# gabefreedman/fastfp

Hardware: NVIDIA H100
Metric: Fp evals/sec (freqs x pulsars x draws) (higher is better)
Workload: dtype f64

## Files before the change

fastfp_b200/csrc/ffp_internal.cuh:

```cuda
#pragma once
#include <cuda_runtime.h>
#include <stdint.h>

#include <atomic>
#include <map>
#include <memory>
#include <string>
#include <type_traits>
#include <vector>

#include "../../include/fastfp_b200.h"

namespace ffp {

constexpr int NWC = 8;
constexpr int NWP = 16;
constexpr int NTC = NWC * 32, NTP = NWP * 32;
constexpr int CTAS_PER_SM = 1;
constexpr int CONSUMER_REGS = 120, PRODUCER_REGS = 56;
constexpr int VST = 16;
constexpr int FLUSH_TOAS = 512;
constexpr int MAX_M = 640;
constexpr int RG_ROWS = 288;
constexpr int MAX_M_WIDE = 2688;
constexpr int MAX_RG = (MAX_M_WIDE + RG_ROWS - 1) / RG_ROWS;

__host__ __device__ inline int row_groups(int m) { return m <= MAX_M ? 1 : (m + RG_ROWS - 1) / RG_ROWS; }
__host__ __device__ inline int row_group_start(int m, int k) {
  const int nb = (m + 7) / 8, g = row_groups(m);
  const int r = 8 * (k * (nb / g) + (k < nb % g ? k : nb % g));
  return r < m ? r : m;
}

inline int sweep_rows(int m, int64_t R, bool blockn) {
  return (m + 7) / 8 * 8 + (int)((R + 7) / 8 * 8) + (blockn ? 8 : 0);
}

template <int NMBW_, int NNB_, int WMW_, int CI_, int NWC_ = ffp::NWC, int NWP_ = ffp::NWP,
          int CREGS_ = CONSUMER_REGS, int PREGS_ = PRODUCER_REGS>
struct SweepCfg {
  static constexpr int NMBW = NMBW_, NNB = NNB_, WMW = WMW_, CI = CI_;
  static constexpr int NWC = NWC_, NWP = NWP_, NTC = NWC_ * 32, NTP = NWP_ * 32, NTHREADS = NTC + NTP;
  static constexpr int CREGS = CREGS_, PREGS = PREGS_;
  static_assert(NTHREADS <= 1024 && NWC % WMW_ == 0, "warp layout");
  static_assert(NTC * CREGS + NTP * PREGS <= NTHREADS * ((65536 / NTHREADS) / 8 * 8), "register pool");
  static constexpr int WNW = NWC / WMW;
  static constexpr int KF = WNW * NNB * 4;
  static constexpr int NMB = NMBW * WMW;
  static constexpr int MP = 8 * NMB;
  static constexpr int KB = CI / 4;
  static constexpr int ST = CI * 2 * KF;
  static constexpr int VEC = 4 * CI;
  static constexpr int GT = CI * MP;
  static constexpr int PK = VEC + GT;
  static constexpr int NX = KF / 8;
  static constexpr int XW = NX >= NWP ? NX / NWP : 1;
  static constexpr int KSPLIT = NX >= ffp::NWP ? 1 : (ffp::NWP / NX < KB ? ffp::NWP / NX : KB);
  static constexpr int KBW = KB / KSPLIT;
  static constexpr int WPG = NX >= NWP ? 1 : (NWP / NX < KSPLIT ? NWP / NX : KSPLIT);
  static constexpr int SPW = KSPLIT / WPG;
  static constexpr int NACTIVE = NX >= NWP ? NWP : NX * WPG;
  static constexpr int NV = PREGS >= 72 ? KBW * XW : 1;
  static constexpr int NACC = 2 * NMBW * NNB;
  static constexpr int NACCX = NACC + 3 * NNB;
  static constexpr int SLAB = NACCX * NTC + 5 * SPW * XW * NTP;
  static constexpr int FLUSH = FLUSH_TOAS / CI;
  static constexpr int SST = ST * 8 * 8 <= 140 * 1024 ? 8 : 4;
  static constexpr int GBUDGET = 214 * 1024 - SST * ST * 8 - VST * VEC * 8;
  static constexpr int GST = GBUDGET / (GT * 8) >= 8 ? 8 : (GBUDGET / (GT * 8) >= 2 ? GBUDGET / (GT * 8) : 2);
  static constexpr int RED = KF * (3 * WMW + 5 * KSPLIT);
  static constexpr size_t SMEM =
      (size_t)(SST * ST + GST * GT + VST * VEC + KF + RED + 2 * (SST + GST + VST)) * 8 + 128;
  static_assert(KB % KSPLIT == 0 && KSPLIT % WPG == 0 && NACTIVE <= NWP && (KBW * XW) % NV == 0,
                "basis-phase mapping");
  static_assert(GST >= 3, "the consumers prefetch across chunk boundaries: three G stages at least");
};

__host__ __device__ inline int g_frag_index(int il, int j, int nmb) {
  return (((il >> 2) * nmb + (j >> 3)) << 5) + (((j & 7) << 2) | (il & 3));
}

struct PulsarMeta {
  int64_t pk_off;
  int64_t L_off;
  int64_t raw_off;
  int64_t T_off;
  int32_t n, m, nch, mpad;
  int32_t mfix, mvar;
  int32_t var_off;
  int32_t ci;
  double tabs_max;
  int64_t dm_off;
  int64_t i8_off;
  int32_t i8_rows;
  int32_t i8_nst;
  double ninv_sum;
};
constexpr int RG_WIDE = 4;

struct KernelCfg {
  int nmbw, nnb, wmw, ci;
  int nwc = NWC;
  int kf() const { return (nwc / wmw) * nnb * 4; }
  int mp() const { return 8 * nmbw * wmw; }
  bool operator<(const KernelCfg& o) const {
    if (nmbw != o.nmbw) return nmbw < o.nmbw;
// ... 260 lines not shown
               const double* dx, const double* dy, const double* dx0, double* d_work, double* d_out,
               cudaStream_t st);
int run_fp64_peak(int kind, int iters, double* tflops, double* ms);

__device__ __forceinline__ uint32_t smem_u32(const void* p) {
  return (uint32_t)__cvta_generic_to_shared(p);
}
__device__ __forceinline__ void mbar_init(uint64_t* bar, int count) {
  asm volatile("mbarrier.init.shared::cta.b64 [%0], %1;" ::"r"(smem_u32(bar)), "r"(count));
}
__device__ __forceinline__ void mbar_expect_tx(uint64_t* bar, uint32_t bytes) {
  asm volatile("mbarrier.arrive.expect_tx.shared::cta.b64 _, [%0], %1;" ::"r"(smem_u32(bar)),
               "r"(bytes)
               : "memory");
}
__device__ __forceinline__ void tma_load_1d(void* dst_smem, const void* src_gmem, uint32_t bytes,
                                            uint64_t* bar) {
  asm volatile(
      "cp.async.bulk.shared::cluster.global.mbarrier::complete_tx::bytes [%0], [%1], %2, [%3];" ::
          "r"(smem_u32(dst_smem)),
      "l"(src_gmem), "r"(bytes), "r"(smem_u32(bar))
      : "memory");
}
__device__ __forceinline__ bool mbar_try_wait(uint64_t* bar, uint32_t parity) {
  uint32_t ok;
  asm volatile(
      "{\n .reg .pred p;\n mbarrier.try_wait.parity.shared::cta.b64 p, [%1], %2;\n"
      " selp.b32 %0, 1, 0, p;\n}"
      : "=r"(ok)
      : "r"(smem_u32(bar)), "r"(parity)
      : "memory");
  return ok != 0;
}
__device__ __forceinline__ void mbar_wait(uint64_t* bar, uint32_t parity) {
  if (mbar_try_wait(bar, parity)) return;
  while (!mbar_try_wait(bar, parity)) __nanosleep(64);
}
__device__ __forceinline__ void mbar_wait_spin(uint64_t* bar, uint32_t parity) {
  while (!mbar_try_wait(bar, parity)) {}
}
__device__ __forceinline__ void mbar_arrive(uint64_t* bar) {
  asm volatile("mbarrier.arrive.shared::cta.b64 _, [%0];" ::"r"(smem_u32(bar)) : "memory");
}
__device__ __forceinline__ void fence_barrier_init() {
  asm volatile("fence.mbarrier_init.release.cluster;" ::: "memory");
}
__device__ __forceinline__ void fence_proxy_async() {
  asm volatile("fence.proxy.async.shared::cta;" ::: "memory");
}

template <int R>
__device__ __forceinline__ void reg_alloc() {
  asm volatile("setmaxnreg.inc.sync.aligned.u32 %0;" ::"n"(R));
}
template <int R>
__device__ __forceinline__ void reg_dealloc() {
  asm volatile("setmaxnreg.dec.sync.aligned.u32 %0;" ::"n"(R));
}

__device__ __forceinline__ void dmma_m8n8k4(double& d0, double& d1, double a, double b) {
  asm("mma.sync.aligned.m8n8k4.row.col.f64.f64.f64.f64 {%0,%1}, {%2}, {%3}, {%0,%1};"
      : "+d"(d0), "+d"(d1)
      : "d"(a), "d"(b));
}
__device__ __forceinline__ void dmma_m16n8k4(double (&d)[4], double a0, double a1, double b) {
  asm("mma.sync.aligned.m16n8k4.row.col.f64.f64.f64.f64 {%0,%1,%2,%3}, {%4,%5}, {%6}, {%0,%1,%2,%3};"
// ... 124 lines not shown
```

fastfp_b200/csrc/fp_sweep_kernel.cuh:

```cuda
#pragma once
#include "ffp_internal.cuh"
#include "ffp_sincos.cuh"

namespace ffp {

enum class SweepMode { Fp, Nmfp, Res };

struct SweepArgs {
  const double* packets;
  const PulsarMeta* meta;
  const int* pidx;
  int ntile_f;
  int nwork;
  const double* freqs;
  int64_t F;
  union {
    FpOut fp;
    NmfpTiles nm;
    ResOut res;
  };
  RowGroupOut rg;
  double* slab;
  unsigned int* counter;
  const unsigned char* done_mask;
// ... 6 lines not shown
#else
#define FFP_DBG(ar, bit) 0
#endif

template <class C>
struct SweepSmem {
  double* Sring;
  double* Gring;
  double* Vring;
  double* fq;
  double* red;
  uint64_t *s_full, *s_empty, *g_full, *g_empty, *v_full, *v_empty;
  __device__ explicit SweepSmem(unsigned char* raw) {
    Sring = reinterpret_cast<double*>(raw);
    Gring = Sring + C::SST * C::ST;
    Vring = Gring + C::GST * C::GT;
    fq = Vring + VST * C::VEC;
    red = fq + C::KF;
    s_full = reinterpret_cast<uint64_t*>(red + C::RED);
    s_empty = s_full + C::SST;
    g_full = s_empty + C::SST;
    g_empty = g_full + C::GST;
    v_full = g_empty + C::GST;
    v_empty = v_full + VST;
  }
};

struct WorkItem {
  int p, ft, nch;
  const double* gpk;
};

template <class C>
__device__ __forceinline__ void producer_loop(const SweepArgs& ar, SweepSmem<C>& sm, volatile int* s_work,
                                              const int pw, const int lane) {
  constexpr int XW = C::XW, SPW = C::SPW, KBW = C::KBW, NV = C::NV;
  const int tidp = pw * 32 + lane;
  const int bk = lane & 3, bf8 = lane >> 2;
  const int bx0 = C::NX >= C::NWP ? pw * XW : pw % C::NX;
  const int bsplit = C::NX >= C::NWP ? 0 : (pw / C::NX) * SPW;
  const int sofs = 2 * lane;
  double* const sl = ar.slab + (size_t)blockIdx.x * C::SLAB + (size_t)C::NACCX * C::NTC + tidp;
  uint32_t g = 0;
  for (;;) {
    __syncthreads();
    const int w = *s_work;
    if (w >= ar.nwork) break;
    const int gp = w / ar.ntile_f;
    const PulsarMeta pm = ar.meta[ar.pidx[gp]];
    const double* gpk = ar.packets + pm.pk_off;
    const int nch = pm.nch;
    auto issue_vec = [&](int c) {
      const uint32_t k = g + (uint32_t)c;
      uint64_t* b = &sm.v_full[k % VST];
      mbar_expect_tx(b, C::VEC * 8);
      tma_load_1d(sm.Vring + (k % VST) * C::VEC, gpk + (size_t)c * C::PK, C::VEC * 8, b);
    };
    if (pw == 0 && lane == 0)
      for (int c = 0; c < VST - 1 && c < nch; ++c) issue_vec(c);
    __syncthreads();
    double omega[XW];
#pragma unroll
    for (int xx = 0; xx < XW; ++xx)
      omega[xx] = __dmul_rn(6.283185307179586, sm.fq[8 * (bx0 + xx) + bf8]);
    bool fast = true;
#pragma unroll
    for (int xx = 0; xx < XW; ++xx) fast = fast && (fabs(omega[xx]) * pm.tabs_max <= 0.999 * FFP_SINCOS_MAX);
    fast = __all_sync(0xffffffffu, fast);
    double s2[SPW][XW][5];
#pragma unroll
    for (int sp = 0; sp < SPW; ++sp)
#pragma unroll
      for (int xx = 0; xx < XW; ++xx)
#pragma unroll
        for (int q = 0; q < 5; ++q) s2[sp][xx][q] = 0.0;
    bool flushed = false;

    for (int c = 0; c < nch; ++c) {
      const uint32_t k = g + (uint32_t)c;
      if (pw == 0 && lane == 0 && c + VST - 2 < nch && c >= 1) {
        if (k >= 2) mbar_wait(&sm.v_empty[(k - 2) % VST], ((k - 2) / VST) & 1u);
        issue_vec(c + VST - 2);
      }
      mbar_wait(&sm.v_full[k % VST], (k / VST) & 1u);
      if (k >= C::SST) mbar_wait(&sm.s_empty[k % C::SST], ((k / C::SST) - 1) & 1u);
      const double* pk = sm.Vring + (k % VST) * C::VEC;
      double* sb = sm.Sring + (k % C::SST) * C::ST + sofs;
      if (!FFP_DBG(ar, 1) && pw < C::NACTIVE) {
#pragma unroll
        for (int sp = 0; sp < SPW; ++sp) {
          const int kb0 = (bsplit + sp) * KBW;
          if (fast) {
#pragma unroll
            for (int e0 = 0; e0 < KBW * XW; e0 += NV) {
              double ph[NV], s[NV], cs[NV], ni[NV], wv[NV];
#pragma unroll
              for (int v = 0; v < NV; ++v) {
                const int i = 4 * (kb0 + (e0 + v) / XW) + bk;
                const double2 tn = *reinterpret_cast<const double2*>(pk + 4 * i);
                ph[v] = __dmul_rn(omega[(e0 + v) % XW], tn.x);
                ni[v] = tn.y;
                wv[v] = pk[4 * i + 2];
// ... 13 lines not shown
              }
            }
          } else {
#pragma unroll 1
            for (int e = 0; e < KBW * XW; ++e) {
              const int kb = kb0 + e / XW, xx = e % XW;
              const int i = 4 * kb + bk;
              const double om = __dmul_rn(6.283185307179586, sm.fq[8 * (bx0 + xx) + bf8]);
              const double ph = __dmul_rn(om, pk[4 * i]);
              double s, cs;
              sincos(ph, &s, &cs);
              const double ni = pk[4 * i + 1], wv = pk[4 * i + 2];
              *reinterpret_cast<double2*>(sb + (kb * C::NX + bx0 + xx) * 64) = make_double2(s, cs);
              const double sn = s * ni, cn = cs * ni;
#pragma unroll
              for (int x2 = 0; x2 < XW; ++x2)
                if (x2 == xx) {
                  s2[sp][x2][0] = fma(sn, s, s2[sp][x2][0]);
                  s2[sp][x2][1] = fma(sn, cs, s2[sp][x2][1]);
                  s2[sp][x2][2] = fma(cn, cs, s2[sp][x2][2]);
                  s2[sp][x2][3] = fma(s, wv, s2[sp][x2][3]);
                  s2[sp][x2][4] = fma(cs, wv, s2[sp][x2][4]);
                }
            }
          }
        }
      }
      __syncwarp();
      if (lane == 0) {
        mbar_arrive(&sm.s_full[k % C::SST]);
        mbar_arrive(&sm.v_empty[k % VST]);
      }
      if ((c + 1) % C::FLUSH == 0 && c + 1 < nch && !FFP_DBG(ar, 4)) {
#pragma unroll
        for (int sp = 0; sp < SPW; ++sp)
#pragma unroll
          for (int xx = 0; xx < XW; ++xx)
#pragma unroll
            for (int q = 0; q < 5; ++q) {
              double* a = sl + (size_t)((sp * XW + xx) * 5 + q) * C::NTP;
              if (flushed) atomicAdd(a, s2[sp][xx][q]);
              else __stcg(a, s2[sp][xx][q]);
              s2[sp][xx][q] = 0.0;
            }
        flushed = true;
      }
    }
    g += (uint32_t)nch;
    if (flushed) __threadfence();
#pragma unroll
    for (int sp = 0; sp < SPW; ++sp)
#pragma unroll
      for (int xx = 0; xx < XW; ++xx)
#pragma unroll
        for (int q = 0; q < 5; ++q) {
          double v = s2[sp][xx][q];
          if (flushed) v += __ldcg(sl + (size_t)((sp * XW + xx) * 5 + q) * C::NTP);
          v += __shfl_xor_sync(0xffffffffu, v, 1);
          v += __shfl_xor_sync(0xffffffffu, v, 2);
          s2[sp][xx][q] = v;
        }
    double* redA = sm.red + C::WMW * C::KF * 3;
    if (bk == 0 && pw < C::NACTIVE) {
#pragma unroll
      for (int sp = 0; sp < SPW; ++sp)
#pragma unroll
        for (int xx = 0; xx < XW; ++xx)
#pragma unroll
          for (int q = 0; q < 5; ++q)
            redA[((bsplit + sp) * C::KF + 8 * (bx0 + xx) + bf8) * 5 + q] = s2[sp][xx][q];
    }
    __syncthreads();
    __syncthreads();
  }
}

template <class C>
__device__ __forceinline__ void res_tail(const ResOut& out, int64_t F, const SweepSmem<C>& sm,
                                         const double (&acc)[C::NMBW][C::NNB / 2][4], const double* redB, int p,
                                         int64_t f0, int m, int wm, int wn, int lane) {
  constexpr int NMBW = C::NMBW, NMT = C::NNB / 2;
  asm volatile("bar.sync 1, %0;" ::"n"(C::NTC) : "memory");
  const int r0 = (m + 7) & ~7;
#pragma unroll
  for (int q = 0; q < NMT; ++q) {
    const int fl = 8 * (wn * NMT + q) + (lane >> 2);
    const int64_t f = f0 + fl;
    if (f >= F) continue;
    const double m00 = redB[fl * 3], m01 = redB[fl * 3 + 1], m11 = redB[fl * 3 + 2], fq = sm.fq[fl];
#pragma unroll
    for (int r = 0; r < NMBW; ++r)
#pragma unroll
    for (int e = 0; e < 2; ++e) {
      const int k = 8 * (wm * NMBW + r) + 2 * (lane & 3) + e - r0;
      if (k < 0 || k >= out.R) continue;
      out.put(k, p, f, F, fq, m00, m01, m11, acc[r][q][e], acc[r][q][2 + e]);
    }
  }
}

template <class C, SweepMode MODE, bool ECORR>
__device__ __forceinline__ void consumer_loop(const SweepArgs& ar, SweepSmem<C>& sm, volatile int* s_work,
                                              const int cw, const int lane) {
  constexpr int NMBW = C::NMBW, NMT = C::NNB / 2;
  static_assert(C::NNB % 2 == 0, "16-row MMA tiles: frequencies in groups of 8");
  const int tid = cw * 32 + lane;
  const int wm = cw / C::WNW, wn = cw - wm * C::WNW;
  double* const sl = ar.slab + (size_t)blockIdx.x * C::SLAB + tid;
  uint32_t g = 0;
  for (;;) {
    if (tid == 0) *s_work = (int)atomicAdd(ar.counter, 1u);
    __syncthreads();
    const int w = *s_work;
    if (w >= ar.nwork) break;
    const int gp = w / ar.ntile_f, ft = w - gp * ar.ntile_f;
    const int p = ar.pidx[gp];
    const PulsarMeta pm = ar.meta[p];
    const double* gpk = ar.packets + pm.pk_off;
    const int nch = pm.nch;
    const int64_t f0 = (int64_t)ft * C::KF;
    auto issue_G = [&](int c) {
      const uint32_t k = g + (uint32_t)c;
      uint64_t* b = &sm.g_full[k % C::GST];
      mbar_expect_tx(b, C::GT * 8);
      tma_load_1d(sm.Gring + (k % C::GST) * C::GT, gpk + (size_t)c * C::PK + C::VEC, C::GT * 8, b);
    };
    if (tid == 0)
      for (int c = 0; c < C::GST - 1 && c < nch; ++c) issue_G(c);
    if (tid < C::KF) sm.fq[tid] = ar.freqs[f0 + tid < ar.F ? f0 + tid : f0];
    __syncthreads();

    double acc[NMBW][NMT][4];
#pragma unroll
    for (int r = 0; r < NMBW; ++r)
#pragma unroll
      for (int q = 0; q < NMT; ++q) acc[r][q][0] = acc[r][q][1] = acc[r][q][2] = acc[r][q][3] = 0.0;
    bool flushed = false;
    double es[NMT][2][3];
#pragma unroll
    for (int q = 0; q < NMT; ++q)
#pragma unroll
      for (int e = 0; e < 2; ++e) es[q][e][0] = es[q][e][1] = es[q][e][2] = 0.0;
    const bool slot_warp = ECORR && wm == C::WMW - 1;
    const unsigned char* dmask = ECORR ? ar.done_mask + pm.dm_off : nullptr;

    double2 a0[NMT];
    double b0[NMBW];
    {
      const uint32_t k = g;
      mbar_wait_spin(&sm.g_full[k % C::GST], (k / C::GST) & 1u);
      mbar_wait_spin(&sm.s_full[k % C::SST], (k / C::SST) & 1u);
      const double* gt = sm.Gring + (k % C::GST) * C::GT + (wm * NMBW) * 32 + lane;
      const double* sb = sm.Sring + (k % C::SST) * C::ST + (wn * NMT) * 64 + 2 * lane;
#pragma unroll
      for (int r = 0; r < NMBW; ++r) b0[r] = gt[r * 32];
#pragma unroll
      for (int q = 0; q < NMT; ++q) a0[q] = *reinterpret_cast<const double2*>(sb + q * 64);
    }
    for (int c = 0; c < nch; ++c) {
      const uint32_t k = g + (uint32_t)c;
      if (tid == 0 && c + C::GST - 2 < nch && c >= 1) {
        if (k >= 2) mbar_wait(&sm.g_empty[(k - 2) % C::GST], ((k - 2) / C::GST) & 1u);
        issue_G(c + C::GST - 2);
      }
      const double* gt = sm.Gring + (k % C::GST) * C::GT + (wm * NMBW) * 32 + lane;
      const double* sb = sm.Sring + (k % C::SST) * C::ST + (wn * NMT) * 64 + 2 * lane;
#pragma unroll
      for (int kb = 0; kb < C::KB; ++kb) {
        double2 a1[NMT];
        double b1[NMBW];
        if (kb + 1 < C::KB) {
// ... 3 lines not shown
          for (int q = 0; q < NMT; ++q) a1[q] = *reinterpret_cast<const double2*>(sb + ((kb + 1) * C::NX + q) * 64);
        } else if (c + 1 < nch) {
          const uint32_t k1 = k + 1;
          mbar_wait_spin(&sm.g_full[k1 % C::GST], (k1 / C::GST) & 1u);
          mbar_wait_spin(&sm.s_full[k1 % C::SST], (k1 / C::SST) & 1u);
          const double* gt1 = sm.Gring + (k1 % C::GST) * C::GT + (wm * NMBW) * 32 + lane;
          const double* sb1 = sm.Sring + (k1 % C::SST) * C::ST + (wn * NMT) * 64 + 2 * lane;
#pragma unroll
          for (int r = 0; r < NMBW; ++r) b1[r] = gt1[r * 32];
#pragma unroll
          for (int q = 0; q < NMT; ++q) a1[q] = *reinterpret_cast<const double2*>(sb1 + q * 64);
        } else {
#pragma unroll
          for (int r = 0; r < NMBW; ++r) b1[r] = 0.0;
#pragma unroll
          for (int q = 0; q < NMT; ++q) a1[q] = make_double2(0.0, 0.0);
        }
        if (!FFP_DBG(ar, 2)) {
#pragma unroll
          for (int r = 0; r < NMBW; ++r)
#pragma unroll
            for (int q = 0; q < NMT; ++q) dmma_m16n8k4(acc[r][q], a0[q].x, a0[q].y, b0[r]);
        }
#pragma unroll
        for (int r = 0; r < NMBW; ++r) b0[r] = b1[r];
#pragma unroll
        for (int q = 0; q < NMT; ++q) a0[q] = a1[q];
      }
      __syncwarp();
      if (lane == 0) {
        mbar_arrive(&sm.g_empty[k % C::GST]);
        mbar_arrive(&sm.s_empty[k % C::SST]);
      }
      if (ECORR && slot_warp) {
        const unsigned dm = (unsigned)dmask[c] >> (2 * (lane & 3));
#pragma unroll
        for (int e = 0; e < 2; ++e)
          if ((dm >> e) & 1u) {
#pragma unroll
            for (int q = 0; q < NMT; ++q) {
              const double ys = acc[NMBW - 1][q][e], yc = acc[NMBW - 1][q][2 + e];
              es[q][e][0] = fma(ys, ys, es[q][e][0]);
              es[q][e][1] = fma(ys, yc, es[q][e][1]);
              es[q][e][2] = fma(yc, yc, es[q][e][2]);
              acc[NMBW - 1][q][e] = acc[NMBW - 1][q][2 + e] = 0.0;
            }
          }
      }
      if ((c + 1) % C::FLUSH == 0 && c + 1 < nch && !FFP_DBG(ar, 4)) {
#pragma unroll
        for (int r = 0; r < NMBW; ++r)
#pragma unroll
          for (int q = 0; q < NMT; ++q)
#pragma unroll
            for (int e = 0; e < 4; ++e) {
              if (ECORR && r == NMBW - 1 && slot_warp) continue;
              double* a = sl + (size_t)((r * NMT + q) * 4 + e) * C::NTC;
              if (flushed) atomicAdd(a, acc[r][q][e]);
              else __stcg(a, acc[r][q][e]);
              acc[r][q][e] = 0.0;
            }
        if (ECORR && slot_warp) {
#pragma unroll
          for (int q = 0; q < NMT; ++q)
#pragma unroll
            for (int e = 0; e < 6; ++e) {
              double* a = sl + (size_t)(C::NACC + q * 6 + e) * C::NTC;
              if (flushed) atomicAdd(a, es[q][e / 3][e % 3]);
              else __stcg(a, es[q][e / 3][e % 3]);
              es[q][e / 3][e % 3] = 0.0;
            }
        }
        flushed = true;
      }
    }
    g += (uint32_t)nch;

    if (flushed) {
      __threadfence();
#pragma unroll
      for (int r = 0; r < NMBW; ++r)
#pragma unroll
        for (int q = 0; q < NMT; ++q)
#pragma unroll
          for (int e = 0; e < 4; ++e)
            if (!(ECORR && r == NMBW - 1 && slot_warp)) acc[r][q][e] += __ldcg(sl + (size_t)((r * NMT + q) * 4 + e) * C::NTC);
      if (ECORR && slot_warp) {
#pragma unroll
        for (int q = 0; q < NMT; ++q)
#pragma unroll
          for (int e = 0; e < 6; ++e) es[q][e / 3][e % 3] += __ldcg(sl + (size_t)(C::NACC + q * 6 + e) * C::NTC);
      }
    }
    const int mfix = pm.mfix;
    double* redB = sm.red;
#pragma unroll
    for (int q = 0; q < NMT; ++q) {
      double ps[2][3] = {{0, 0, 0}, {0, 0, 0}};
#pragma unroll
      for (int r = 0; r < NMBW; ++r)
#pragma unroll
      for (int e = 0; e < 2; ++e) {
        const int j = 8 * (wm * NMBW + r) + 2 * (lane & 3) + e;
        const double ys = acc[r][q][e], yc = acc[r][q][2 + e];
        if (j < mfix) {
          ps[e][0] = fma(ys, ys, ps[e][0]);
          ps[e][1] = fma(ys, yc, ps[e][1]);
          ps[e][2] = fma(yc, yc, ps[e][2]);
        } else if (MODE == SweepMode::Nmfp && j < pm.m) {
          const int64_t f = f0 + 8 * (wn * NMT + q) + (lane >> 2);
          if (f < ar.F) {
            double* z = ar.nm.z(p, f, (ar.F + 31) >> 5, j - mfix + (ar.nm.mvpad - pm.mvar));
            z[0] = ys;
            z[16] = yc;
          }
        }
      }
#pragma unroll
      for (int k = 0; k < 3; ++k) {
        if (ECORR && slot_warp) {
          ps[0][k] += es[q][0][k];
          ps[1][k] += es[q][1][k];
        }
        double v = ps[0][k] + ps[1][k];
        v += __shfl_xor_sync(0xffffffffu, v, 1);
        v += __shfl_xor_sync(0xffffffffu, v, 2);
        if ((lane & 3) == 0) redB[(wm * C::KF + 8 * (wn * NMT + q) + (lane >> 2)) * 3 + k] = v;
      }
    }
    __syncthreads();
    const int64_t fidx = f0 + tid;
    if (tid < C::KF && fidx < ar.F) {
      const double* redA = sm.red + C::WMW * C::KF * 3;
      double b[3] = {0, 0, 0}, a[5] = {0, 0, 0, 0, 0};
      for (int w2 = 0; w2 < C::WMW; ++w2)
#pragma unroll
        for (int k = 0; k < 3; ++k) b[k] += redB[(w2 * C::KF + tid) * 3 + k];
      for (int g2 = 0; g2 < C::KSPLIT; ++g2)
#pragma unroll
        for (int k = 0; k < 5; ++k) a[k] += redA[(g2 * C::KF + tid) * 5 + k];
      if (MODE == SweepMode::Fp) {
        if (p < ar.rg.first) ar.fp.put(p, fidx, ar.F, sm.fq[tid], a[0] - b[0], a[1] - b[1], a[2] - b[2], a[3], a[4]);
        else ar.rg.put(p, fidx, ar.F, sm.fq[tid], a, b);
      }
      if (MODE == SweepMode::Nmfp) ar.nm.put_a(p, fidx, (ar.F + 31) >> 5, a[0] - b[0], a[1] - b[1], a[2] - b[2], a[3], a[4]);
      if (MODE == SweepMode::Res) {
        redB[tid * 3 + 0] = a[0] - b[0];
        redB[tid * 3 + 1] = a[1] - b[1];
        redB[tid * 3 + 2] = a[2] - b[2];
        ar.res.put_m(p, fidx, sm.fq[tid], a[0] - b[0], a[1] - b[1], a[2] - b[2]);
      }
    }
    if (MODE == SweepMode::Res) res_tail<C>(ar.res, ar.F, sm, acc, redB, p, f0, pm.m, wm, wn, lane);
    __syncthreads();
  }
}

template <class C, SweepMode MODE, bool ECORR>
__global__ void __launch_bounds__(C::NTHREADS, CTAS_PER_SM) fp_sweep_kernel(const SweepArgs ar) {
  extern __shared__ __align__(128) unsigned char smem_raw[];
  SweepSmem<C> sm(smem_raw);
  __shared__ int s_work;
  const int tid = threadIdx.x, lane = tid & 31, wid = tid >> 5;
  if (tid == 0) {
    for (int s = 0; s < C::SST; ++s) { mbar_init(&sm.s_full[s], C::NWP); mbar_init(&sm.s_empty[s], C::NWC); }
    for (int s = 0; s < C::GST; ++s) { mbar_init(&sm.g_full[s], 1); mbar_init(&sm.g_empty[s], C::NWC); }
    for (int s = 0; s < VST; ++s) { mbar_init(&sm.v_full[s], 1); mbar_init(&sm.v_empty[s], C::NWP); }
    fence_barrier_init();
  }
  __syncthreads();
  if (wid < C::NWC) {
    reg_alloc<C::CREGS>();
    consumer_loop<C, MODE, ECORR>(ar, sm, &s_work, wid, lane);
  } else {
    reg_dealloc<C::PREGS>();
    producer_loop<C>(ar, sm, &s_work, wid - C::NWC, lane);
  }
}

template <class C, SweepMode MODE, bool ECORR>
int launch_sweep_cfg(const fastfp_pack* pk, const GroupView& g, const SweepArgs& base, cudaStream_t st) {
  static bool attr_done[64] = {};
  if (!attr_done[pk->device & 63]) {
    FFP_CUDA(cudaFuncSetAttribute(fp_sweep_kernel<C, MODE, ECORR>,
                                  cudaFuncAttributeMaxDynamicSharedMemorySize, (int)C::SMEM));
    attr_done[pk->device & 63] = true;
  }
  SweepArgs a = base;
  a.pidx = g.pidx;
  const int64_t ntile = (a.F + C::KF - 1) / C::KF;
  const int64_t nwork = ntile * g.count;
  if (nwork > 0x7fffffffLL) { set_error("frequency batch too large for one launch"); return -1; }
  a.ntile_f = (int)ntile;
  a.nwork = (int)nwork;
  const int64_t resident = (int64_t)CTAS_PER_SM * pk->num_sms;
  const unsigned grid = (unsigned)(nwork < resident ? nwork : resident);
  FFP_CUDA(cudaMemsetAsync(a.counter, 0, sizeof(unsigned int), st));
  fp_sweep_kernel<C, MODE, ECORR><<<grid, C::NTHREADS, C::SMEM, st>>>(a);
  g_launches += 1;
  FFP_CUDA(cudaGetLastError());
  return 0;
}

int dispatch_sweep_w1(const fastfp_pack*, const GroupView&, const SweepArgs&, SweepMode, cudaStream_t);
// ... 23 lines not shown
```

fastfp_b200/csrc/fp_sweep_w2.cu:

```cuda
#include "fp_sweep_kernel.cuh"
namespace ffp {
#define FFP_SWEEP_CASE_W2(NMBWv) FFP_SWEEP_CASE_W(NMBWv, 2, 1, 32, 8, 8, 168, 88)
int dispatch_sweep_w2(const fastfp_pack* pk, const GroupView& g, const SweepArgs& a, SweepMode mode, cudaStream_t st) {
  FFP_SWEEP_CASE_W2(6) FFP_SWEEP_CASE_W2(7) FFP_SWEEP_CASE_W2(8) FFP_SWEEP_CASE_W2(9) FFP_SWEEP_CASE_W2(10)
  set_error("no sweep kernel for this configuration (w2)");
  return -3;
}
}
```

Measured before the change: 11.62 million.

## Add fused single-role sweep kernel replacing producer/consumer split for w2 configs

Adds a fused kernel path, used when NWP is zero. Each of the 8 warps computes its own sincos basis values in registers and feeds them straight into the DMMA, so the producer warps and the shared-memory S ring are gone. TMA refill is issued by thread 0 with a non-blocking test_wait lookahead. Sincos for the next chunk is software-pipelined against the MMA of the current chunk. The w2 dispatch switches to this config with 255 registers per thread, trading warp specialization and latency hiding for no smem staging and more registers.

Result: slower. 10.15 million, median of 6 (-12.7%).

```diff
diff --git a/fastfp_b200/csrc/ffp_internal.cuh b/fastfp_b200/csrc/ffp_internal.cuh
--- a/fastfp_b200/csrc/ffp_internal.cuh
+++ b/fastfp_b200/csrc/ffp_internal.cuh
@@ -54,24 +54,26 @@
   static constexpr int GT = CI * MP;
   static constexpr int PK = VEC + GT;
   static constexpr int NX = KF / 8;
-  static constexpr int XW = NX >= NWP ? NX / NWP : 1;
+  static constexpr bool FUSED = NWP == 0;
+  static constexpr int NSW = FUSED ? NWC : NWP, NTS = NSW * 32;
+  static constexpr int XW = NX >= NSW ? NX / NSW : 1;
   static constexpr int KSPLIT = NX >= ffp::NWP ? 1 : (ffp::NWP / NX < KB ? ffp::NWP / NX : KB);
   static constexpr int KBW = KB / KSPLIT;
-  static constexpr int WPG = NX >= NWP ? 1 : (NWP / NX < KSPLIT ? NWP / NX : KSPLIT);
+  static constexpr int WPG = NX >= NSW ? 1 : (NSW / NX < KSPLIT ? NSW / NX : KSPLIT);
   static constexpr int SPW = KSPLIT / WPG;
-  static constexpr int NACTIVE = NX >= NWP ? NWP : NX * WPG;
-  static constexpr int NV = PREGS >= 72 ? KBW * XW : 1;
+  static constexpr int NACTIVE = NX >= NSW ? NSW : NX * WPG;
+  static constexpr int NV = (FUSED ? CREGS : PREGS) >= 72 ? KBW * XW : 1;
   static constexpr int NACC = 2 * NMBW * NNB;
   static constexpr int NACCX = NACC + 3 * NNB;
-  static constexpr int SLAB = NACCX * NTC + 5 * SPW * XW * NTP;
+  static constexpr int SLAB = NACCX * NTC + 5 * SPW * XW * NTS;
   static constexpr int FLUSH = FLUSH_TOAS / CI;
-  static constexpr int SST = ST * 8 * 8 <= 140 * 1024 ? 8 : 4;
+  static constexpr int SST = FUSED ? 0 : ST * 8 * 8 <= 140 * 1024 ? 8 : 4;
   static constexpr int GBUDGET = 214 * 1024 - SST * ST * 8 - VST * VEC * 8;
   static constexpr int GST = GBUDGET / (GT * 8) >= 8 ? 8 : (GBUDGET / (GT * 8) >= 2 ? GBUDGET / (GT * 8) : 2);
   static constexpr int RED = KF * (3 * WMW + 5 * KSPLIT);
   static constexpr size_t SMEM =
       (size_t)(SST * ST + GST * GT + VST * VEC + KF + RED + 2 * (SST + GST + VST)) * 8 + 128;
-  static_assert(KB % KSPLIT == 0 && KSPLIT % WPG == 0 && NACTIVE <= NWP && (KBW * XW) % NV == 0,
+  static_assert(KB % KSPLIT == 0 && KSPLIT % WPG == 0 && NACTIVE <= NSW && (KBW * XW) % NV == 0,
                 "basis-phase mapping");
   static_assert(GST >= 3, "the consumers prefetch across chunk boundaries: three G stages at least");
 };
@@ -398,6 +400,16 @@
       : "memory");
   return ok != 0;
 }
+__device__ __forceinline__ bool mbar_test_wait(uint64_t* bar, uint32_t parity) {
+  uint32_t ok;
+  asm volatile(
+      "{\n .reg .pred p;\n mbarrier.test_wait.parity.shared::cta.b64 p, [%1], %2;\n"
+      " selp.b32 %0, 1, 0, p;\n}"
+      : "=r"(ok)
+      : "r"(smem_u32(bar)), "r"(parity)
+      : "memory");
+  return ok != 0;
+}
 __device__ __forceinline__ void mbar_wait(uint64_t* bar, uint32_t parity) {
   if (mbar_try_wait(bar, parity)) return;
   while (!mbar_try_wait(bar, parity)) __nanosleep(64);
diff --git a/fastfp_b200/csrc/fp_sweep_kernel.cuh b/fastfp_b200/csrc/fp_sweep_kernel.cuh
--- a/fastfp_b200/csrc/fp_sweep_kernel.cuh
+++ b/fastfp_b200/csrc/fp_sweep_kernel.cuh
@@ -62,6 +62,102 @@
 };
 
 template <class C>
+using SweepAcc = double[C::NMBW][C::NNB / 2][4];
+template <class C>
+using EpochSums = double[C::NNB / 2][2][3];
+template <class C>
+using ScalarSums = double[C::SPW][C::XW][5];
+
+template <class C>
+__device__ __forceinline__ void flush_sums(ScalarSums<C>& s2, double* sl, bool flushed) {
+#pragma unroll
+  for (int sp = 0; sp < C::SPW; ++sp)
+#pragma unroll
+    for (int xx = 0; xx < C::XW; ++xx)
+#pragma unroll
+      for (int q = 0; q < 5; ++q) {
+        double* a = sl + (size_t)((sp * C::XW + xx) * 5 + q) * C::NTS;
+        if (flushed) atomicAdd(a, s2[sp][xx][q]);
+        else __stcg(a, s2[sp][xx][q]);
+        s2[sp][xx][q] = 0.0;
+      }
+}
+
+template <class C>
+__device__ __forceinline__ void publish_sums(SweepSmem<C>& sm, ScalarSums<C>& s2, const double* sl, bool flushed,
+                                             int bsplit, int bx0, int lane, bool active) {
+  if (flushed) __threadfence();
+#pragma unroll
+  for (int sp = 0; sp < C::SPW; ++sp)
+#pragma unroll
+    for (int xx = 0; xx < C::XW; ++xx)
+#pragma unroll
+      for (int q = 0; q < 5; ++q) {
+        double v = s2[sp][xx][q];
+        if (flushed) v += __ldcg(sl + (size_t)((sp * C::XW + xx) * 5 + q) * C::NTS);
+        v += __shfl_xor_sync(0xffffffffu, v, 1);
+        v += __shfl_xor_sync(0xffffffffu, v, 2);
+        s2[sp][xx][q] = v;
+      }
+  double* redA = sm.red + C::WMW * C::KF * 3;
+  if ((lane & 3) == 0 && active) {
+#pragma unroll
+    for (int sp = 0; sp < C::SPW; ++sp)
+#pragma unroll
+      for (int xx = 0; xx < C::XW; ++xx)
+#pragma unroll
+        for (int q = 0; q < 5; ++q)
+          redA[((bsplit + sp) * C::KF + 8 * (bx0 + xx) + (lane >> 2)) * 5 + q] = s2[sp][xx][q];
+  }
+}
+
+template <class C>
+__device__ __forceinline__ void fold_epochs(SweepAcc<C>& acc, EpochSums<C>& es, unsigned dm, int lane) {
+  dm >>= 2 * (lane & 3);
+#pragma unroll
+  for (int e = 0; e < 2; ++e)
+    if ((dm >> e) & 1u) {
+#pragma unroll
+      for (int q = 0; q < C::NNB / 2; ++q) {
+        const double ys = acc[C::NMBW - 1][q][e], yc = acc[C::NMBW - 1][q][2 + e];
+        es[q][e][0] = fma(ys, ys, es[q][e][0]);
+        es[q][e][1] = fma(ys, yc, es[q][e][1]);
+        es[q][e][2] = fma(yc, yc, es[q][e][2]);
+        acc[C::NMBW - 1][q][e] = acc[C::NMBW - 1][q][2 + e] = 0.0;
+      }
+    }
+}
+
+template <class C, bool ECORR>
+__device__ __forceinline__ void flush_acc(SweepAcc<C>& acc, EpochSums<C>& es, double* sl, bool flushed,
+                                          bool slot_warp) {
+  constexpr int NMBW = C::NMBW, NMT = C::NNB / 2;
+#pragma unroll
+  for (int r = 0; r < NMBW; ++r)
+#pragma unroll
+    for (int q = 0; q < NMT; ++q)
+#pragma unroll
+      for (int e = 0; e < 4; ++e) {
+        if (ECORR && r == NMBW - 1 && slot_warp) continue;
+        double* a = sl + (size_t)((r * NMT + q) * 4 + e) * C::NTC;
+        if (flushed) atomicAdd(a, acc[r][q][e]);
+        else __stcg(a, acc[r][q][e]);
+        acc[r][q][e] = 0.0;
+      }
+  if (ECORR && slot_warp) {
+#pragma unroll
+    for (int q = 0; q < NMT; ++q)
+#pragma unroll
+      for (int e = 0; e < 6; ++e) {
+        double* a = sl + (size_t)(C::NACC + q * 6 + e) * C::NTC;
+        if (flushed) atomicAdd(a, es[q][e / 3][e % 3]);
+        else __stcg(a, es[q][e / 3][e % 3]);
+        es[q][e / 3][e % 3] = 0.0;
+      }
+  }
+}
+
+template <class C>
 __device__ __forceinline__ void producer_loop(const SweepArgs& ar, SweepSmem<C>& sm, volatile int* s_work,
                                               const int pw, const int lane) {
   constexpr int XW = C::XW, SPW = C::SPW, KBW = C::KBW, NV = C::NV;
@@ -97,7 +193,7 @@
 #pragma unroll
     for (int xx = 0; xx < XW; ++xx) fast = fast && (fabs(omega[xx]) * pm.tabs_max <= 0.999 * FFP_SINCOS_MAX);
     fast = __all_sync(0xffffffffu, fast);
-    double s2[SPW][XW][5];
+    ScalarSums<C> s2;
 #pragma unroll
     for (int sp = 0; sp < SPW; ++sp)
 #pragma unroll
@@ -177,44 +273,12 @@
         mbar_arrive(&sm.v_empty[k % VST]);
       }
       if ((c + 1) % C::FLUSH == 0 && c + 1 < nch && !FFP_DBG(ar, 4)) {
-#pragma unroll
-        for (int sp = 0; sp < SPW; ++sp)
-#pragma unroll
-          for (int xx = 0; xx < XW; ++xx)
-#pragma unroll
-            for (int q = 0; q < 5; ++q) {
-              double* a = sl + (size_t)((sp * XW + xx) * 5 + q) * C::NTP;
-              if (flushed) atomicAdd(a, s2[sp][xx][q]);
-              else __stcg(a, s2[sp][xx][q]);
-              s2[sp][xx][q] = 0.0;
-            }
+        flush_sums<C>(s2, sl, flushed);
         flushed = true;
       }
     }
     g += (uint32_t)nch;
-    if (flushed) __threadfence();
-#pragma unroll
-    for (int sp = 0; sp < SPW; ++sp)
-#pragma unroll
-      for (int xx = 0; xx < XW; ++xx)
-#pragma unroll
-        for (int q = 0; q < 5; ++q) {
-          double v = s2[sp][xx][q];
-          if (flushed) v += __ldcg(sl + (size_t)((sp * XW + xx) * 5 + q) * C::NTP);
-          v += __shfl_xor_sync(0xffffffffu, v, 1);
-          v += __shfl_xor_sync(0xffffffffu, v, 2);
-          s2[sp][xx][q] = v;
-        }
-    double* redA = sm.red + C::WMW * C::KF * 3;
-    if (bk == 0 && pw < C::NACTIVE) {
-#pragma unroll
-      for (int sp = 0; sp < SPW; ++sp)
-#pragma unroll
-        for (int xx = 0; xx < XW; ++xx)
-#pragma unroll
-          for (int q = 0; q < 5; ++q)
-            redA[((bsplit + sp) * C::KF + 8 * (bx0 + xx) + bf8) * 5 + q] = s2[sp][xx][q];
-    }
+    publish_sums<C>(sm, s2, sl, flushed, bsplit, bx0, lane, pw < C::NACTIVE);
     __syncthreads();
     __syncthreads();
   }
@@ -242,6 +306,91 @@
       out.put(k, p, f, F, fq, m00, m01, m11, acc[r][q][e], acc[r][q][2 + e]);
     }
   }
+}
+
+template <class C, SweepMode MODE, bool ECORR>
+__device__ __forceinline__ void sweep_epilogue(const SweepArgs& ar, SweepSmem<C>& sm, SweepAcc<C>& acc,
+                                               EpochSums<C>& es, const double* sl, bool flushed, const PulsarMeta& pm,
+                                               int p, int64_t f0, int wm, int wn, int lane) {
+  constexpr int NMBW = C::NMBW, NMT = C::NNB / 2;
+  const bool slot_warp = ECORR && wm == C::WMW - 1;
+  if (flushed) {
+    __threadfence();
+#pragma unroll
+    for (int r = 0; r < NMBW; ++r)
+#pragma unroll
+      for (int q = 0; q < NMT; ++q)
+#pragma unroll
+        for (int e = 0; e < 4; ++e)
+          if (!(ECORR && r == NMBW - 1 && slot_warp)) acc[r][q][e] += __ldcg(sl + (size_t)((r * NMT + q) * 4 + e) * C::NTC);
+    if (ECORR && slot_warp) {
+#pragma unroll
+      for (int q = 0; q < NMT; ++q)
+#pragma unroll
+        for (int e = 0; e < 6; ++e) es[q][e / 3][e % 3] += __ldcg(sl + (size_t)(C::NACC + q * 6 + e) * C::NTC);
+    }
+  }
+  const int mfix = pm.mfix;
+  double* redB = sm.red;
+#pragma unroll
+  for (int q = 0; q < NMT; ++q) {
+    double ps[2][3] = {{0, 0, 0}, {0, 0, 0}};
+#pragma unroll
+    for (int r = 0; r < NMBW; ++r)
+#pragma unroll
+    for (int e = 0; e < 2; ++e) {
+      const int j = 8 * (wm * NMBW + r) + 2 * (lane & 3) + e;
+      const double ys = acc[r][q][e], yc = acc[r][q][2 + e];
+      if (j < mfix) {
+        ps[e][0] = fma(ys, ys, ps[e][0]);
+        ps[e][1] = fma(ys, yc, ps[e][1]);
+        ps[e][2] = fma(yc, yc, ps[e][2]);
+      } else if (MODE == SweepMode::Nmfp && j < pm.m) {
+        const int64_t f = f0 + 8 * (wn * NMT + q) + (lane >> 2);
+        if (f < ar.F) {
+          double* z = ar.nm.z(p, f, (ar.F + 31) >> 5, j - mfix + (ar.nm.mvpad - pm.mvar));
+          z[0] = ys;
+          z[16] = yc;
+        }
+      }
+    }
+#pragma unroll
+    for (int k = 0; k < 3; ++k) {
+      if (ECORR && slot_warp) {
+        ps[0][k] += es[q][0][k];
+        ps[1][k] += es[q][1][k];
+      }
+      double v = ps[0][k] + ps[1][k];
+      v += __shfl_xor_sync(0xffffffffu, v, 1);
+      v += __shfl_xor_sync(0xffffffffu, v, 2);
+      if ((lane & 3) == 0) redB[(wm * C::KF + 8 * (wn * NMT + q) + (lane >> 2)) * 3 + k] = v;
+    }
+  }
+  __syncthreads();
+  const int tid = (wm * C::WNW + wn) * 32 + lane;
+  const int64_t fidx = f0 + tid;
+  if (tid < C::KF && fidx < ar.F) {
+    const double* redA = sm.red + C::WMW * C::KF * 3;
+    double b[3] = {0, 0, 0}, a[5] = {0, 0, 0, 0, 0};
+    for (int w2 = 0; w2 < C::WMW; ++w2)
+#pragma unroll
+      for (int k = 0; k < 3; ++k) b[k] += redB[(w2 * C::KF + tid) * 3 + k];
+    for (int g2 = 0; g2 < C::KSPLIT; ++g2)
+#pragma unroll
+      for (int k = 0; k < 5; ++k) a[k] += redA[(g2 * C::KF + tid) * 5 + k];
+    if (MODE == SweepMode::Fp) {
+      if (p < ar.rg.first) ar.fp.put(p, fidx, ar.F, sm.fq[tid], a[0] - b[0], a[1] - b[1], a[2] - b[2], a[3], a[4]);
+      else ar.rg.put(p, fidx, ar.F, sm.fq[tid], a, b);
+    }
+    if (MODE == SweepMode::Nmfp) ar.nm.put_a(p, fidx, (ar.F + 31) >> 5, a[0] - b[0], a[1] - b[1], a[2] - b[2], a[3], a[4]);
+    if (MODE == SweepMode::Res) {
+      redB[tid * 3 + 0] = a[0] - b[0];
+      redB[tid * 3 + 1] = a[1] - b[1];
+      redB[tid * 3 + 2] = a[2] - b[2];
+      ar.res.put_m(p, fidx, sm.fq[tid], a[0] - b[0], a[1] - b[1], a[2] - b[2]);
+    }
+  }
+  if (MODE == SweepMode::Res) res_tail<C>(ar.res, ar.F, sm, acc, redB, p, f0, pm.m, wm, wn, lane);
 }
 
 template <class C, SweepMode MODE, bool ECORR>
@@ -275,13 +424,13 @@
     if (tid < C::KF) sm.fq[tid] = ar.freqs[f0 + tid < ar.F ? f0 + tid : f0];
     __syncthreads();
 
-    double acc[NMBW][NMT][4];
+    SweepAcc<C> acc;
 #pragma unroll
     for (int r = 0; r < NMBW; ++r)
 #pragma unroll
       for (int q = 0; q < NMT; ++q) acc[r][q][0] = acc[r][q][1] = acc[r][q][2] = acc[r][q][3] = 0.0;
     bool flushed = false;
-    double es[NMT][2][3];
+    EpochSums<C> es;
 #pragma unroll
     for (int q = 0; q < NMT; ++q)
 #pragma unroll
@@ -351,126 +500,173 @@
         mbar_arrive(&sm.g_empty[k % C::GST]);
         mbar_arrive(&sm.s_empty[k % C::SST]);
       }
-      if (ECORR && slot_warp) {
-        const unsigned dm = (unsigned)dmask[c] >> (2 * (lane & 3));
-#pragma unroll
-        for (int e = 0; e < 2; ++e)
-          if ((dm >> e) & 1u) {
-#pragma unroll
-            for (int q = 0; q < NMT; ++q) {
-              const double ys = acc[NMBW - 1][q][e], yc = acc[NMBW - 1][q][2 + e];
-              es[q][e][0] = fma(ys, ys, es[q][e][0]);
-              es[q][e][1] = fma(ys, yc, es[q][e][1]);
-              es[q][e][2] = fma(yc, yc, es[q][e][2]);
-              acc[NMBW - 1][q][e] = acc[NMBW - 1][q][2 + e] = 0.0;
-            }
-          }
-      }
+      if (ECORR && slot_warp) fold_epochs<C>(acc, es, dmask[c], lane);
       if ((c + 1) % C::FLUSH == 0 && c + 1 < nch && !FFP_DBG(ar, 4)) {
-#pragma unroll
-        for (int r = 0; r < NMBW; ++r)
-#pragma unroll
-          for (int q = 0; q < NMT; ++q)
-#pragma unroll
-            for (int e = 0; e < 4; ++e) {
-              if (ECORR && r == NMBW - 1 && slot_warp) continue;
-              double* a = sl + (size_t)((r * NMT + q) * 4 + e) * C::NTC;
-              if (flushed) atomicAdd(a, acc[r][q][e]);
-              else __stcg(a, acc[r][q][e]);
-              acc[r][q][e] = 0.0;
-            }
-        if (ECORR && slot_warp) {
-#pragma unroll
-          for (int q = 0; q < NMT; ++q)
-#pragma unroll
-            for (int e = 0; e < 6; ++e) {
-              double* a = sl + (size_t)(C::NACC + q * 6 + e) * C::NTC;
-              if (flushed) atomicAdd(a, es[q][e / 3][e % 3]);
-              else __stcg(a, es[q][e / 3][e % 3]);
-              es[q][e / 3][e % 3] = 0.0;
-            }
-        }
+        flush_acc<C, ECORR>(acc, es, sl, flushed, slot_warp);
         flushed = true;
       }
     }
     g += (uint32_t)nch;
-
-    if (flushed) {
-      __threadfence();
-#pragma unroll
-      for (int r = 0; r < NMBW; ++r)
-#pragma unroll
-        for (int q = 0; q < NMT; ++q)
-#pragma unroll
-          for (int e = 0; e < 4; ++e)
-            if (!(ECORR && r == NMBW - 1 && slot_warp)) acc[r][q][e] += __ldcg(sl + (size_t)((r * NMT + q) * 4 + e) * C::NTC);
-      if (ECORR && slot_warp) {
-#pragma unroll
-        for (int q = 0; q < NMT; ++q)
-#pragma unroll
-          for (int e = 0; e < 6; ++e) es[q][e / 3][e % 3] += __ldcg(sl + (size_t)(C::NACC + q * 6 + e) * C::NTC);
-      }
-    }
-    const int mfix = pm.mfix;
-    double* redB = sm.red;
-#pragma unroll
-    for (int q = 0; q < NMT; ++q) {
-      double ps[2][3] = {{0, 0, 0}, {0, 0, 0}};
-#pragma unroll
-      for (int r = 0; r < NMBW; ++r)
-#pragma unroll
-      for (int e = 0; e < 2; ++e) {
-        const int j = 8 * (wm * NMBW + r) + 2 * (lane & 3) + e;
-        const double ys = acc[r][q][e], yc = acc[r][q][2 + e];
-        if (j < mfix) {
-          ps[e][0] = fma(ys, ys, ps[e][0]);
-          ps[e][1] = fma(ys, yc, ps[e][1]);
-          ps[e][2] = fma(yc, yc, ps[e][2]);
-        } else if (MODE == SweepMode::Nmfp && j < pm.m) {
-          const int64_t f = f0 + 8 * (wn * NMT + q) + (lane >> 2);
-          if (f < ar.F) {
-            double* z = ar.nm.z(p, f, (ar.F + 31) >> 5, j - mfix + (ar.nm.mvpad - pm.mvar));
-            z[0] = ys;
-            z[16] = yc;
+    sweep_epilogue<C, MODE, ECORR>(ar, sm, acc, es, sl, flushed, pm, p, f0, wm, wn, lane);
+    __syncthreads();
+  }
+}
+
+
+template <int NV>
+__device__ __noinline__ void sincos_cold(const double (&x)[NV], double (&s)[NV], double (&c)[NV]) {
+#pragma unroll
+  for (int v = 0; v < NV; ++v) sincos(x[v], &s[v], &c[v]);
+}
+
+template <class C, bool FAST>
+__device__ __forceinline__ void fused_sincos(const double* pk, int bk, double omega, double (&s)[C::KB],
+                                             double (&cs)[C::KB], double (&a0)[5], double (&a1)[5]) {
+  constexpr int NV = C::KB, h = 0;
+  double ph[NV], ni[NV], wv[NV];
+#pragma unroll
+  for (int v = 0; v < NV; ++v) {
+    const int i = 4 * (h * NV + v) + bk;
+    const double2 tn = *reinterpret_cast<const double2*>(pk + 4 * i);
+    ph[v] = __dmul_rn(omega, tn.x);
+    ni[v] = tn.y;
+    wv[v] = pk[4 * i + 2];
+  }
+  if (FAST) {
+    sincos_cw_n<NV>(ph, s, cs);
+  } else {
+    sincos_cold<NV>(ph, s, cs);
+  }
+#pragma unroll
+  for (int v = 0; v < NV; ++v) {
+    double (&a)[5] = v < C::KBW ? a0 : a1;
+    const double sn = s[v] * ni[v], cn = cs[v] * ni[v];
+    a[0] = fma(sn, s[v], a[0]);
+    a[1] = fma(sn, cs[v], a[1]);
+    a[2] = fma(cn, cs[v], a[2]);
+    a[3] = fma(s[v], wv[v], a[3]);
+    a[4] = fma(cs[v], wv[v], a[4]);
+  }
+}
+
+template <class C>
+__device__ __forceinline__ void fused_mma(SweepAcc<C>& acc, const double* gt, const double (&s)[C::KB],
+                                          const double (&cs)[C::KB], bool on) {
+#pragma unroll
+  for (int v = 0; v < C::KB; ++v) {
+    const int kb = v;
+    double b[C::NMBW];
+#pragma unroll
+    for (int r = 0; r < C::NMBW; ++r) b[r] = gt[(kb * C::NMB + r) * 32];
+    if (on) {
+#pragma unroll
+      for (int r = 0; r < C::NMBW; ++r) dmma_m16n8k4(acc[r][0], s[v], cs[v], b[r]);
+    }
+  }
+}
+
+template <class C, SweepMode MODE, bool ECORR>
+__device__ __forceinline__ void fused_loop(const SweepArgs& ar, SweepSmem<C>& sm, volatile int* s_work, const int cw,
+                                           const int lane) {
+  static_assert(C::WMW == 1 && C::NNB == 2 && C::NX == C::NWC && C::XW == 1 && C::KSPLIT == 2 && C::SPW == 2 &&
+                    C::NV == C::KBW,
+                "fused: warp cw owns frequency group cw and both halves of the chunk's k-blocks");
+  static_assert(VST >= C::GST, "fused: one empty barrier for both rings");
+  constexpr int NMBW = C::NMBW, KBW = C::KBW;
+  const int tid = cw * 32 + lane, bk = lane & 3;
+  double* const sl = ar.slab + (size_t)blockIdx.x * C::SLAB + tid;
+  double* const sl2 = sl + (size_t)C::NACCX * C::NTC;
+  uint32_t g = 0;
+  for (;;) {
+    if (tid == 0) *s_work = (int)atomicAdd(ar.counter, 1u);
+    __syncthreads();
+    const int w = *s_work;
+    if (w >= ar.nwork) break;
+    const int gp = w / ar.ntile_f, ft = w - gp * ar.ntile_f;
+    const int p = ar.pidx[gp];
+    const int nch = ar.meta[p].nch;
+    const int64_t f0 = (int64_t)ft * C::KF;
+    if (tid < C::KF) sm.fq[tid] = ar.freqs[f0 + tid < ar.F ? f0 + tid : f0];
+    __syncthreads();
+    const double omega = __dmul_rn(6.283185307179586, sm.fq[8 * cw + (lane >> 2)]);
+    const bool fast = __all_sync(0xffffffffu, fabs(omega) * ar.meta[p].tabs_max <= 0.999 * FFP_SINCOS_MAX);
+    SweepAcc<C> acc;
+#pragma unroll
+    for (int r = 0; r < NMBW; ++r) acc[r][0][0] = acc[r][0][1] = acc[r][0][2] = acc[r][0][3] = 0.0;
+    EpochSums<C> es;
+#pragma unroll
+    for (int e = 0; e < 2; ++e) es[0][e][0] = es[0][e][1] = es[0][e][2] = 0.0;
+    ScalarSums<C> s2;
+#pragma unroll
+    for (int q = 0; q < 5; ++q) s2[0][0][q] = s2[1][0][q] = 0.0;
+    bool flushed = false;
+    const unsigned char* dmask = ECORR ? ar.done_mask + ar.meta[p].dm_off : nullptr;
+    const bool math = !FFP_DBG(ar, 1), mma = !FFP_DBG(ar, 2);
+    const double* gpk = ar.packets + ar.meta[p].pk_off;
+    int issued = 0;
+    auto refill = [&](int c) {
+      for (; issued < nch && issued < c + C::GST; ++issued) {
+        const uint32_t k = g + (uint32_t)issued;
+        if (k >= C::GST) {
+          uint64_t* e = &sm.g_empty[k % C::GST];
+          const uint32_t par = ((k / C::GST) - 1) & 1u;
+          if (issued > c + 1) {
+            if (!mbar_test_wait(e, par)) break;
+          } else {
+            mbar_wait_spin(e, par);
           }
         }
-      }
-#pragma unroll
-      for (int k = 0; k < 3; ++k) {
-        if (ECORR && slot_warp) {
-          ps[0][k] += es[q][0][k];
-          ps[1][k] += es[q][1][k];
+        uint64_t* v = &sm.v_full[k % VST];
+        mbar_expect_tx(v, C::VEC * 8);
+        tma_load_1d(sm.Vring + (k % VST) * C::VEC, gpk + (size_t)issued * C::PK, C::VEC * 8, v);
+        uint64_t* b = &sm.g_full[k % C::GST];
+        mbar_expect_tx(b, C::GT * 8);
+        tma_load_1d(sm.Gring + (k % C::GST) * C::GT, gpk + (size_t)issued * C::PK + C::VEC, C::GT * 8, b);
+      }
+    };
+
+    auto sweep = [&](auto fast_c) {
+      constexpr bool FAST = decltype(fast_c)::value;
+      double sA[C::KB], cA[C::KB];
+#pragma unroll
+      for (int v = 0; v < C::KB; ++v) sA[v] = cA[v] = 0.0;
+      auto vec = [&](uint32_t k) { return sm.Vring + (k % VST) * C::VEC; };
+      if (tid == 0) refill(0);
+      mbar_wait_spin(&sm.v_full[g % VST], (g / VST) & 1u);
+      if (math) fused_sincos<C, FAST>(vec(g), bk, omega, sA, cA, s2[0][0], s2[1][0]);
+      for (int c = 0; c < nch; ++c) {
+        const uint32_t k = g + (uint32_t)c;
+        const double* gt = sm.Gring + (k % C::GST) * C::GT + lane;
+        const bool flush = (c + 1) % C::FLUSH == 0 && c + 1 < nch && !FFP_DBG(ar, 4);
+        if (flush) flush_sums<C>(s2, sl2, flushed);
+        if (tid == 0 && c > 0) refill(c);
+        mbar_wait_spin(&sm.g_full[k % C::GST], (k / C::GST) & 1u);
+        double sB[C::KB], cB[C::KB];
+        if (c + 1 < nch) {
+          mbar_wait_spin(&sm.v_full[(k + 1) % VST], ((k + 1) / VST) & 1u);
+          if (math) fused_sincos<C, FAST>(vec(k + 1), bk, omega, sB, cB, s2[0][0], s2[1][0]);
         }
-        double v = ps[0][k] + ps[1][k];
-        v += __shfl_xor_sync(0xffffffffu, v, 1);
-        v += __shfl_xor_sync(0xffffffffu, v, 2);
-        if ((lane & 3) == 0) redB[(wm * C::KF + 8 * (wn * NMT + q) + (lane >> 2)) * 3 + k] = v;
-      }
-    }
-    __syncthreads();
-    const int64_t fidx = f0 + tid;
-    if (tid < C::KF && fidx < ar.F) {
-      const double* redA = sm.red + C::WMW * C::KF * 3;
-      double b[3] = {0, 0, 0}, a[5] = {0, 0, 0, 0, 0};
-      for (int w2 = 0; w2 < C::WMW; ++w2)
-#pragma unroll
-        for (int k = 0; k < 3; ++k) b[k] += redB[(w2 * C::KF + tid) * 3 + k];
-      for (int g2 = 0; g2 < C::KSPLIT; ++g2)
-#pragma unroll
-        for (int k = 0; k < 5; ++k) a[k] += redA[(g2 * C::KF + tid) * 5 + k];
-      if (MODE == SweepMode::Fp) {
-        if (p < ar.rg.first) ar.fp.put(p, fidx, ar.F, sm.fq[tid], a[0] - b[0], a[1] - b[1], a[2] - b[2], a[3], a[4]);
-        else ar.rg.put(p, fidx, ar.F, sm.fq[tid], a, b);
-      }
-      if (MODE == SweepMode::Nmfp) ar.nm.put_a(p, fidx, (ar.F + 31) >> 5, a[0] - b[0], a[1] - b[1], a[2] - b[2], a[3], a[4]);
-      if (MODE == SweepMode::Res) {
-        redB[tid * 3 + 0] = a[0] - b[0];
-        redB[tid * 3 + 1] = a[1] - b[1];
-        redB[tid * 3 + 2] = a[2] - b[2];
-        ar.res.put_m(p, fidx, sm.fq[tid], a[0] - b[0], a[1] - b[1], a[2] - b[2]);
-      }
-    }
-    if (MODE == SweepMode::Res) res_tail<C>(ar.res, ar.F, sm, acc, redB, p, f0, pm.m, wm, wn, lane);
+        fused_mma<C>(acc, gt, sA, cA, mma);
+        __syncwarp();
+        if (lane == 0) mbar_arrive(&sm.g_empty[k % C::GST]);
+        if (ECORR) fold_epochs<C>(acc, es, dmask[c], lane);
+        if (flush) {
+          flush_acc<C, ECORR>(acc, es, sl, flushed, ECORR);
+          flushed = true;
+        }
+#pragma unroll
+        for (int v = 0; v < C::KB; ++v) {
+          sA[v] = sB[v];
+          cA[v] = cB[v];
+        }
+      }
+    };
+    if (fast) sweep(std::true_type{});
+    else sweep(std::false_type{});
+    g += (uint32_t)nch;
+    publish_sums<C>(sm, s2, sl2, flushed, 0, cw, lane, true);
+    const PulsarMeta pm = ar.meta[p];
+    sweep_epilogue<C, MODE, ECORR>(ar, sm, acc, es, sl, flushed, pm, p, f0, 0, cw, lane);
     __syncthreads();
   }
 }
@@ -484,11 +680,12 @@
   if (tid == 0) {
     for (int s = 0; s < C::SST; ++s) { mbar_init(&sm.s_full[s], C::NWP); mbar_init(&sm.s_empty[s], C::NWC); }
     for (int s = 0; s < C::GST; ++s) { mbar_init(&sm.g_full[s], 1); mbar_init(&sm.g_empty[s], C::NWC); }
-    for (int s = 0; s < VST; ++s) { mbar_init(&sm.v_full[s], 1); mbar_init(&sm.v_empty[s], C::NWP); }
+    for (int s = 0; s < VST; ++s) { mbar_init(&sm.v_full[s], 1); mbar_init(&sm.v_empty[s], C::NSW); }
     fence_barrier_init();
   }
   __syncthreads();
-  if (wid < C::NWC) {
+  if constexpr (C::FUSED) fused_loop<C, MODE, ECORR>(ar, sm, &s_work, wid, lane);
+  else if (wid < C::NWC) {
     reg_alloc<C::CREGS>();
     consumer_loop<C, MODE, ECORR>(ar, sm, &s_work, wid, lane);
   } else {
diff --git a/fastfp_b200/csrc/fp_sweep_w2.cu b/fastfp_b200/csrc/fp_sweep_w2.cu
--- a/fastfp_b200/csrc/fp_sweep_w2.cu
+++ b/fastfp_b200/csrc/fp_sweep_w2.cu
@@ -1,6 +1,6 @@
 #include "fp_sweep_kernel.cuh"
 namespace ffp {
-#define FFP_SWEEP_CASE_W2(NMBWv) FFP_SWEEP_CASE_W(NMBWv, 2, 1, 32, 8, 8, 168, 88)
+#define FFP_SWEEP_CASE_W2(NMBWv) FFP_SWEEP_CASE_W(NMBWv, 2, 1, 32, 8, 0, 255, 0)
 int dispatch_sweep_w2(const fastfp_pack* pk, const GroupView& g, const SweepArgs& a, SweepMode mode, cudaStream_t st) {
   FFP_SWEEP_CASE_W2(6) FFP_SWEEP_CASE_W2(7) FFP_SWEEP_CASE_W2(8) FFP_SWEEP_CASE_W2(9) FFP_SWEEP_CASE_W2(10)
   set_error("no sweep kernel for this configuration (w2)");
```
